# dgrzech/ir-sgmcmc

Measured on AMD Instinct MI355X. Metric: SG-MCMC transitions/sec (full _SGLD_transition), higher is better.
Workload: dtype f32; 1 GPU; 256^3 synthetic pair, SVF_3D 12 steps, GMM(K=4)/LCC(s=1) + virtual decimation, RegLoss_L2 w=1.4, Sobolev s=3, uniform noise 0.1, SGLD lr 0.4, Philox noise; init=identity, chains=1, parallelism=1 independent chain(s)

## Files before the change

include/irsgmcmc.h:

```cpp
#ifndef IRSGMCMC_H
#define IRSGMCMC_H

#include <stddef.h>
#include <stdint.h>

#ifdef __cplusplus
extern "C" {
#endif
#pragma GCC visibility push(default)

#define IRS_MAX_COMPONENTS 8
#define IRS_MAX_CHAINS 8
#define IRS_MAX_HALF_WIDTH 4
#define IRS_MAX_LABELS 64
#define IRS_HAUSDORFF_MAX_PERCENTILES 4

enum { IRS_DATA_GMM_LCC = 0, IRS_DATA_SSD = 1 };
enum { IRS_REG_L2 = 0, IRS_REG_LOGNORMAL = 1, IRS_REG_STUDENT = 2, IRS_REG_LOGNORMAL_L2 = 3 };


int irs_perturb_smooth(const float* v, const float* sigma, const float* eps, float tau, const float* kernel, int s,
                       int C, int D, int H, int W, float* tmp, float* out, uint64_t seed, uint64_t iteration,
                       void* stream);

// ... 242 lines not shown
void irs_destroy(irs_ctx* ctx);
size_t irs_workspace_bytes(const irs_ctx* ctx);
int irs_velocity_dims(const irs_ctx* ctx, int32_t out[3]);

int irs_set_fixed(irs_ctx* ctx, const float* fixed_im, int fixed_chains, void* stream);
int irs_get_state(irs_ctx* ctx, irs_state* out, void* stream);
int irs_set_state(irs_ctx* ctx, const irs_state* in, void* stream);
int irs_get_scalars(irs_ctx* ctx, irs_scalars* out, void* stream);

int irs_gmm_init(irs_ctx* ctx, const irs_io* io, const float* v_sample, int warm_up, void* stream);

int irs_transition(irs_ctx* ctx, const irs_io* io, void* stream);

int irs_flush(irs_ctx* ctx, void* stream);
int irs_recovered_transitions(const irs_ctx* ctx, uint64_t* out);

typedef struct irs_timings {
    float total_ms;
    float exp_fwd_ms;
    float exp_bwd_kernel_ms;
    float exp_bwd_total_ms;
    float smooth_ms;
    float data_ms;
    float update_ms;
    float exp_bwd_primary_avg_ms;
} irs_timings;
int irs_transition_timed(irs_ctx* ctx, const irs_io* io, void* stream, irs_timings* out);

typedef struct irs_comm irs_comm;
#define IRS_COMM_ID_BYTES 128
// ... 95 lines not shown
```

ir_sgmcmc_amd/_lib.py:

```python
import ctypes as C
import os

import torch

_HERE = os.path.dirname(os.path.abspath(__file__))
LIB_PATH = os.environ.get('IRS_LIB') or os.path.join(_HERE, 'csrc', 'libirsgmcmc.so')

IRS_MAX_COMPONENTS = 8
IRS_MAX_CHAINS = 8
IRS_MAX_HALF_WIDTH = 4
IRS_MAX_LABELS = 64
IRS_HAUSDORFF_MAX_PERCENTILES = 4
IRS_LABEL_BINS = 10
IRS_JACOBIAN_SUMMARY_INTS, IRS_JACOBIAN_SUMMARY_FLOATS = 4, 5
IRS_JACOBIAN_WS_BYTES = 1024 * (IRS_JACOBIAN_SUMMARY_INTS + IRS_JACOBIAN_SUMMARY_FLOATS) * 8
IRS_COVARIANCE_SUMMARY_INTS, IRS_COVARIANCE_SUMMARY_FLOATS = 2, 8
IRS_COVARIANCE_WS_BYTES = 1024 * (IRS_COVARIANCE_SUMMARY_INTS + IRS_COVARIANCE_SUMMARY_FLOATS) * 8
IRS_QUANTILE_MIN_BINS, IRS_QUANTILE_MAX_BINS, IRS_QUANTILE_MAX_PROBS, IRS_QUANTILE_MAX_RECORDS = 4, 256, 8, 65535
IRS_QUANTILE_SUMMARY_INTS, IRS_QUANTILE_SUMMARY_FLOATS = 3, 5
IRS_QUANTILE_WS_BYTES = 1024 * (IRS_QUANTILE_SUMMARY_INTS + IRS_QUANTILE_SUMMARY_FLOATS) * 8
IRS_ICE_SUMMARY_INTS, IRS_ICE_SUMMARY_FLOATS = 2, 3
IRS_ICE_WS_BYTES = IRS_MAX_CHAINS * 1024 * (IRS_ICE_SUMMARY_INTS + IRS_ICE_SUMMARY_FLOATS) * 8
IRS_ICE_MAP_SUMMARY_INTS, IRS_ICE_MAP_SUMMARY_FLOATS = 3, 3
IRS_ICE_MAP_WS_BYTES = 1024 * (IRS_ICE_MAP_SUMMARY_INTS + IRS_ICE_MAP_SUMMARY_FLOATS) * 8
# ... 159 lines not shown
                             C.c_size_t, _P],
    'irs_local_similarity_update': [_P, _I, _I, _I, _I, _P, _P, _P, _I, _P],
    'irs_local_similarity_finalize': [_P, _P, _P, _P, _I, _I, _I, _P, _P, _P, C.c_size_t, _P],
    'irs_create': [C.POINTER(IrsConfig), C.POINTER(_P)],
    'irs_destroy': [_P],
    'irs_workspace_bytes': [_P],
    'irs_velocity_dims': [_P, C.POINTER(C.c_int32 * 3)],
    'irs_set_fixed': [_P, _P, _I, _P],
    'irs_get_state': [_P, C.POINTER(IrsState), _P],
    'irs_set_state': [_P, C.POINTER(IrsState), _P],
    'irs_get_scalars': [_P, C.POINTER(IrsScalars), _P],
    'irs_gmm_init': [_P, C.POINTER(IrsIO), _P, _I, _P],
    'irs_transition': [_P, C.POINTER(IrsIO), _P],
    'irs_flush': [_P, _P],
    'irs_recovered_transitions': [_P, C.POINTER(C.c_uint64)],
    'irs_transition_timed': [_P, C.POINTER(IrsIO), _P, C.POINTER(IrsTimings)],
    'irs_comm_unique_id': [C.POINTER(C.c_uint8 * IRS_COMM_ID_BYTES)],
    'irs_comm_create_rccl': [C.POINTER(C.c_uint8 * IRS_COMM_ID_BYTES), _I, _I, C.POINTER(_P)],
    'irs_comm_create_ipc': [C.c_char_p, _I, _I, C.POINTER(_P)],
    'irs_comm_create_callbacks': [EXCHANGE_FN, ALLREDUCE_FN, _P, _I, _I, C.POINTER(_P)],
    'irs_comm_destroy': [_P],
    'irs_comm_probe': [_P, C.c_size_t, C.c_size_t, _I, _P, C.POINTER(C.c_double * 2)],
    'irs_comm_describe': [_P, C.c_char_p, C.c_size_t],
    'irs_comm_rank': [_P],
    'irs_comm_world': [_P],
    'irs_comm_selftest': [_P, _P],
    'irs_slab_plan_layout': [C.POINTER(IrsConfig), C.POINTER(IrsSlabConfig), _I, _I, C.POINTER(IrsSlabLayout)],
    'irs_slab_create': [C.POINTER(IrsConfig), C.POINTER(IrsSlabConfig), _P, C.POINTER(_P)],
    'irs_slab_get_layout': [_P, C.POINTER(IrsSlabLayout)],
    'irs_slab_transition': [_P, C.POINTER(IrsIO), _P],
# ... 65 lines not shown
```

ir_sgmcmc_amd/csrc/api_ctx.hip:

```cpp
#include <math.h>
#include <string.h>

#include <new>

#include "api_checks.h"
#include "comm.h"

using namespace irs;

static size_t align_up(size_t x) { return (x + 255) & ~(size_t)255; }

static bool is_capturing(hipStream_t st) {
    hipStreamCaptureStatus cap = hipStreamCaptureStatusNone;
    (void)hipStreamIsCapturing(st, &cap);
    return cap != hipStreamCaptureStatusNone;
}


int irs::create_ctx(const irs_config* cfg, const SlabInfo* sl, irs_ctx** out) {
    if (!cfg || !out) return fail("irs_create: null argument");
    const int D = cfg->dims[0], H = cfg->dims[1], W = cfg->dims[2], C = cfg->no_chains;
    if (!dims_ok(C, D, H, W) || !chain_count_ok(C)) return fail("irs_create: bad dims / chains (C <= %d)", IRS_MAX_CHAINS);
    if (cfg->no_steps < 1 || cfg->no_steps > 30) return fail("irs_create: no_steps out of range");
    if (cfg->sobolev_s < 0 || cfg->sobolev_s > IRS_MAX_HALF_WIDTH) return fail("irs_create: sobolev_s out of range");
// ... 4 lines not shown
    } else if (!(cfg->ssd_sigma > 0.0f)) return fail("irs_create: ssd_sigma must be positive");
    if (cfg->reg_loss < IRS_REG_L2 || cfg->reg_loss > IRS_REG_LOGNORMAL_L2) return fail("irs_create: unknown regulariser");
    if ((cfg->reg_loss == IRS_REG_STUDENT || cfg->reg_loss == IRS_REG_LOGNORMAL_L2) && cfg->reg_learnable)
        return fail("irs_create: RegLoss_Student / RegLoss_LogNormal_L2 have no learnable parameters");
    if (cfg->reg_loss == IRS_REG_STUDENT && !(cfg->w_reg_prior_rate > 0.0 && cfg->w_reg_prior_shape > 0.0))
        return fail("irs_create: RegLoss_Student needs a0 > 0 and b0 > 0 (w_reg_prior_shape / w_reg_prior_rate)");
    const bool any_cps = cfg->cps[0] || cfg->cps[1] || cfg->cps[2];
    if (any_cps && (cfg->cps[0] < 1 || cfg->cps[1] < 1 || cfg->cps[2] < 1 || cfg->cps[0] > 8 || cfg->cps[1] > 8 || cfg->cps[2] > 8))
        return fail("irs_create: control point spacing must be 1..8 on every axis");

    irs_ctx* c = new (std::nothrow) irs_ctx();
    if (!c) return fail("irs_create: out of host memory");
    memset((void*)c, 0, sizeof(*c));
    context_born();
    c->kn = global_knobs();
    c->cfg = *cfg;
    c->C = C;
    c->vol = make_vol(D, H, W);
    if (sl && sl->on) {
        c->sl = *sl;
        c->vol.V = (int64_t)(sl->hi - sl->lo) * H * W;
    }
    c->ffd = any_cps;
    c->volv = c->ffd ? make_vol(control_points(D, cfg->cps[0]), control_points(H, cfg->cps[1]), control_points(W, cfg->cps[2]))
                     : c->vol;
    c->sob.s = cfg->sobolev_s;
    for (int i = 0; i <= 2 * cfg->sobolev_s; ++i) c->sob.k[i] = cfg->sobolev_kernel[i];
    if (c->ffd)
        for (int a = 0; a < 3; ++a) c->spl[a] = make_spline(cfg->cps[a]);

// ... 39 lines not shown
    const size_t o_steps = take(fieldI * cfg->no_steps);
    const size_t o_tmpA = take(fieldV > ffd_tmp ? fieldV : ffd_tmp);
    const size_t o_tmpB = take(fieldV);
    const size_t o_vs = take(fieldV);
    const size_t o_gA = take(fieldI), o_gB = take(fieldI);
    const bool third = sl && sl->on && sl->world > 1;
    const size_t o_gC = third ? take(fieldI) : 0;
    const size_t o_warped = take(imageI), o_z = take(imageI), o_sig = take(imageI), o_fhat = take(imageI), o_gM = take(imageI);
    const size_t o_dense = take(c->ffd ? fieldI : 0);
    const size_t o_stat = take(sizeof(double) * kMaxPartialBlocks * kStatVals);
    const size_t o_energy = take(sizeof(double) * kMaxPartialBlocks * IRS_MAX_CHAINS);
    const size_t o_nll = take(sizeof(double) * (size_t)c->nll_blocks * C);
    const size_t o_sums = take(sizeof(double) * (kStatVals + 2 * IRS_MAX_CHAINS));
    const size_t o_dmax = take(sizeof(unsigned) * 4 * IRS_MAX_CHAINS * 32);
    const size_t o_cmm = take(coarse_minmax_bytes(c->vol, C));
    const size_t o_state = take(sizeof(DevState));
    c->slab_bytes = off;
    if (hipMalloc((void**)&c->slab, off) != hipSuccess) {
        irs_destroy(c);
        return fail("irs_create: hipMalloc of %zu workspace bytes failed", off);
    }
    if (c->sl.on) (void)hipMemset(c->slab, 0, off);
    c->steps = (float*)(c->slab + o_steps);
    c->tmpA = (float*)(c->slab + o_tmpA);
    c->tmpB = (float*)(c->slab + o_tmpB);
    c->vs = (float*)(c->slab + o_vs);
    c->gA = (float*)(c->slab + o_gA);
    c->gB = (float*)(c->slab + o_gB);
    c->gC = third ? (float*)(c->slab + o_gC) : nullptr;
    c->warped = (float*)(c->slab + o_warped);
    c->z = (float*)(c->slab + o_z);
    c->sigM = (float*)(c->slab + o_sig);
    c->fhat = (float*)(c->slab + o_fhat);
    c->gM = (float*)(c->slab + o_gM);
    c->dense = c->ffd ? (float*)(c->slab + o_dense) : nullptr;
    c->stat_partials = (double*)(c->slab + o_stat);
    c->energy_partials = (double*)(c->slab + o_energy);
    c->nll_partials = (double*)(c->slab + o_nll);
    c->stat_sum = (double*)(c->slab + o_sums);
    c->energy_sum = c->stat_sum + kStatVals;
    c->nll_sum = c->energy_sum + IRS_MAX_CHAINS;
    c->dmax = (unsigned*)(c->slab + o_dmax);
    c->cmm = (float*)(c->slab + o_cmm);
    c->state = (DevState*)(c->slab + o_state);

    if (ensure_lin_tables(c->lin, D, H, W, nullptr)) {
        irs_destroy(c);
        return fail("irs_create: identity grid allocation failed");
    }
    DevState init;
    memset(&init, 0, sizeof(init));
    init.K = d.K;
    init.mode = d.mode;
    init.ssd_inv_sigma = cfg->data_loss == IRS_DATA_SSD ? 1.0f / cfg->ssd_sigma : 0.0f;
    if (cfg->reg_loss == IRS_REG_L2 || cfg->reg_loss == IRS_REG_LOGNORMAL_L2) init.st.reg_param[0] = log((double)cfg->w_reg);
    for (int ch = 0; ch < IRS_MAX_CHAINS; ++ch) init.sc.alpha[ch] = 1.0;
    hipError_t e = hipMemcpy(c->state, &init, sizeof(init), hipMemcpyHostToDevice);
    if (e == hipSuccess) {
// ... 251 lines not shown
        if (overlap && ch + 1 < C) {
            HIP_TRY(hipEventRecord(c->ev_side[2 * ch], st));
            HIP_TRY(hipStreamWaitEvent(c->side, c->ev_side[2 * ch], 0));
            ds = c->side;
        }
        launch_data_bwd(cfg.data_loss, f, 0, zc, c->sigM + (int64_t)ch * vol.V, mask, 0, nullptr, c->state, ch,
                        c->gM + (int64_t)ch * vol.V, c->nll_partials + (int64_t)ch * c->nll_blocks, cfg.lcc_s, 1, vol, ds, c->nll_seg_C);
        if (ds != st) HIP_TRY(hipEventRecord(c->ev_side[2 * ch + 1], c->side));
    }
    if (batch)
        launch_data_bwd(cfg.data_loss, c->fhat, c->fhat_chains == 1 ? 0 : vol.V, z, c->sigM, io->mask, io->mask_chains == 1 ? 0 : vol.V, nullptr,
                        c->state, 0, c->gM, c->nll_partials, cfg.lcc_s, C, vol, st, c->nll_seg_C);
    if (!fuse_warp_bwd)
        launch_warp_bwd(io->moving_im, io->moving_chains == 1 ? 0 : vol.V, d_last, io->unif,
                        cfg.uniform_alpha > 0.0f ? cfg.uniform_alpha : 0.0f, c->gM, c->gA, C, vol, lin, cfg.seed, 0, it, st);
    LAUNCH_CHECK();
    if (timed) HIP_TRY(hipEventRecord(c->ev[3], st));
    const float* dense = c->ffd ? c->dense : vs;
    float* g0 = nullptr;
    {
        const float* G = c->gA;
        float* bufs[2] = {c->gB, c->gA};
        int cur = 0;
        for (int k = cfg.no_steps - 1; k >= 0; --k) {
            float* out = bufs[cur];
            const float* dk = k == 0 ? dense : c->steps + (int64_t)(k - 1) * field;
            if (timed) HIP_TRY(hipEventRecord(c->ev_bwd[2 * k], st));
            const unsigned* dm = c->dmax + (int64_t)k * C * 4;
            const float* gscale = fuse_warp_bwd && k == cfg.no_steps - 1 ? c->gM : nullptr;
            const int lay = bwd_lay(c, k) | (gscale ? 2 : 0);
            const bool sa = k < 32 && skip_any[k], s2 = k < 32 && skip_r2[k];
            const int gr = global_knobs().lds_from <= 2 ? 1 : 2;
            launch_exp_step_bwd_march(G, dk, out, k == 0, cfg.no_steps, C, vol, lin, dm, (s2 || (gr == 1 && !sa)) ? 1 : 2, sa, gscale, lay,
                                      timed ? c->ev_bwd[2 * k + 1] : nullptr, st);
            if (!sa) launch_exp_step_bwd_lds(G, dk, out, k == 0, cfg.no_steps, C, vol, lin, dm, 2, gr, gscale, lay, c->cmm, st);
            G = out;
            cur ^= 1;
        }
        g0 = const_cast<float*>(G);
    }
    if (timed) HIP_TRY(hipEventRecord(c->ev[4], st));
    float s[3];
    prescale_factors(vol, cfg.no_steps, s);
    if (c->ffd) {
        float* scaled = g0 == c->gA ? c->gB : c->gA;
        launch_scale_channels(g0, scaled, s[0], s[1], s[2], C, vol, st);
        const int G[3] = {volv.D, volv.H, volv.W};
        ffd_adjoint(scaled, c->tmpB, c->tmpA, C, vol, G, c->spl, st);
        launch_sgld_update(io->v, io->sigma, c->tmpB, vs, c->state, cfg.lr, 1.0f, 1.0f, 1.0f, io->grad_v, C, volv, st,
// ... 64 lines not shown
            if (enqueue_transition(c, &c->last_io, st, 0, true)) return 1;
        }
    }
    return fail("irs_flush: transitions keep failing");
}

int irs_flush(irs_ctx* c, void* stream) {
    if (!c) return fail("irs_flush: null argument");
    if (c->sl.on) return irs::slab_flush(c, (hipStream_t)stream);
    return flush_impl(c, (hipStream_t)stream);
}

int irs_recovered_transitions(const irs_ctx* c, uint64_t* out) {
    if (!c || !out) return fail("irs_recovered_transitions: null argument");
    *out = c->fails_total;
    return 0;
}

int irs_transition(irs_ctx* c, const irs_io* io, void* stream) { return transition_impl(c, io, (hipStream_t)stream, 0); }

int irs_transition_timed(irs_ctx* c, const irs_io* io, void* stream, irs_timings* out) {
    if (!out) return fail("irs_transition_timed: null output");
    if (c && c->cfg.no_steps > 32) return fail("irs_transition_timed: at most 32 steps");
    if (transition_impl(c, io, (hipStream_t)stream, 1)) return 1;
    HIP_TRY(hipEventSynchronize(c->ev[5]));
    memset(out, 0, sizeof(*out));
    HIP_TRY(hipEventElapsedTime(&out->total_ms, c->ev[0], c->ev[5]));
    HIP_TRY(hipEventElapsedTime(&out->smooth_ms, c->ev[0], c->ev[1]));
    HIP_TRY(hipEventElapsedTime(&out->exp_fwd_ms, c->ev[1], c->ev[2]));
    HIP_TRY(hipEventElapsedTime(&out->data_ms, c->ev[2], c->ev[3]));
// ... 13 lines not shown
```

ir_sgmcmc_amd/csrc/ctx.h:

```cpp
#pragma once
#include <stdlib.h>
#include <string.h>

#include "kernels.h"
#include "scalar_kernels.h"

struct irs_comm;

namespace irs {

int fail(const char* fmt, ...);

#define HIP_TRY(expr)                                                                               \
    do {                                                                                            \
        hipError_t e_ = (expr);                                                                     \
        if (e_ != hipSuccess) return irs::fail("%s failed: %s", #expr, hipGetErrorString(e_));      \
    } while (0)

#define LAUNCH_CHECK()                                                                              \
    do {                                                                                            \
        hipError_t e_ = hipGetLastError();                                                          \
        if (e_ != hipSuccess) return irs::fail("kernel launch failed: %s", hipGetErrorString(e_)); \
    } while (0)

// ... 14 lines not shown
struct irs_ctx {
    irs_config cfg;
    irs::DevCfg dcfg;
    irs::Vol vol, volv;
    bool ffd;
    int C;
    irs::LinTables lin;
    irs::Taps sob;
    irs::SplineTaps spl[3];
    char* slab;
    size_t slab_bytes;
    float *steps, *tmpA, *tmpB, *vs, *gA, *gB, *gC, *warped, *z, *sigM, *fhat, *gM, *dense;
    double *stat_partials, *energy_partials, *nll_partials;
    double *stat_sum, *energy_sum, *nll_sum;
    unsigned* dmax;
    float* cmm;
    unsigned* hint = nullptr;
    irs::DevState* state;
    int fhat_chains;
    bool fixed_set;
    int nll_blocks;
    int nll_seg_C;
    hipEvent_t ev[8];
    hipEvent_t ev_bwd[64];
    hipEvent_t ra_ev[4];
    hipStream_t side = nullptr;
    hipEvent_t ev_side[2 * IRS_MAX_CHAINS] = {};
    uint64_t n_enqueued = 0;
    irs::Knobs kn;
    bool dmax_clean = false;
// ... 119 lines not shown
```

ir_sgmcmc_amd/csrc/exp_kernels.hip:

```cpp
#include "kernels.h"

#include <type_traits>

namespace irs {

#ifndef IRS_ETX
#define IRS_ETX 32
#define IRS_ETY 8
#define IRS_ETZ 8
#endif
constexpr int ETX = IRS_ETX, ETY = IRS_ETY, ETZ = IRS_ETZ, ETN = ETX * ETY * ETZ;
constexpr int kExpBlock = 512;

struct Scale3L {
    float nm1[3];
    float rnm1[3];
    float inv_pow;
};

typedef float F3 __attribute__((ext_vector_type(3)));
__device__ __forceinline__ F3 ld3g(const float* __restrict__ p) {
    F3 v;
    __builtin_memcpy(&v, p, 12);
    return v;
// ... 725 lines not shown
    }
}

#ifdef IRS_BWD_TRACE
__device__ unsigned long long g_bwd_trace[8 * 64];
extern "C" __attribute__((visibility("default"))) int irs_debug_bwd_trace(unsigned long long* out) {
    return hipMemcpyFromSymbol(out, HIP_SYMBOL(g_bwd_trace), sizeof(g_bwd_trace)) == hipSuccess ? 0 : 1;
}
#define IRS_BT(slot)                                                                                  \
    do {                                                                                              \
        if (btrace_on && btrace_it < 64) g_bwd_trace[btrace_it * 8 + (slot)] = wall_clock64();        \
    } while (0)
#else
#define IRS_BT(slot)
#endif
template <bool PRESCALE, int R>
__device__ __forceinline__ void exp_bwd_march_tile(const float* __restrict__ G, const float* __restrict__ dk,
                                                   float* __restrict__ gout, const Vol vol, const Lin lin, const Scale3L sc,
                                                   const unsigned* __restrict__ dmax, const int seg_len, const int nseg,
                                                   const int r_lo, const int own_rest, const int swz_run, const int tile_id,
                                                   const dim3 tiles, const float* __restrict__ gscale, const int lay) {
    using M = March<PRESCALE, R>;
    constexpr int NP = M::NP, PX = M::PX, PN = M::PN, NIT = M::NIT;
    constexpr int NPQ = R == 2 ? 1 : NP;
    __shared__ float2 q_xy[NPQ * PN], q_zg[NPQ * PN], q_g[NPQ * PN], q_d[NP * PN];
    __shared__ float q_dz[NP * PN];
    const int tile_ = xcd_swizzle_runs(tile_id, (int)(tiles.x * tiles.y * tiles.z), swz_run);
    const int tbx = tile_ % tiles.x, tby = (tile_ / tiles.x) % tiles.y, tbz = tile_ / (tiles.x * tiles.y);
    const int chain = tbz / nseg, seg = tbz % nseg;
    const int hs = max(max((int)floorf(__uint_as_float(dmax[chain * 4 + 0])), (int)floorf(__uint_as_float(dmax[chain * 4 + 1]))),
                       (int)floorf(__uint_as_float(dmax[chain * 4 + 2]))) + 1;
    if (hs <= r_lo || (hs > R && !(R == 2 && own_rest))) return;
    const int ox = tbx * MTX, oy = tby * MTY;
    int z0, z1;
    seg_range(vol, seg, seg_len, z0, z1);
    const int64_t V = vol.V;
    const int64_t cb = (int64_t)chain * 3 * V;
    auto run = [&]() {
    const Lay3 LD = lay3(lay & 1, V), LG = lay3(lay & 2, V), LO = lay3(lay & 4, V);
    if (R == 2 && hs > R) {
        const int gx = ox + (int)(threadIdx.x % MTX), gy = oy + (int)(threadIdx.x / MTX);
        if (gx < vol.W && gy < vol.H)
            exp_bwd_generic_column<PRESCALE>(G + cb, LG, gscale ? gscale + (int64_t)chain * V : nullptr, dk + cb, LD, gout + cb, LO, vol,
                                             lin, sc, gx, gy, z0, z1, hs);
        return;
    }
    const float* __restrict__ dx_ = dk + cb;
    const float* __restrict__ dy_ = dx_ + LD.cs;
    const float* __restrict__ dz_ = dy_ + LD.cs;
    const float* __restrict__ Gx_ = G + cb;
// ... 263 lines not shown
    };
    run();
}

template <bool PRESCALE, int R>
__global__ __launch_bounds__(kMarchBlock, R == 1 ? IRS_MARCH_WAVES : IRS_MARCH_WAVES_R2) void exp_bwd_march_kernel(
    const float* __restrict__ G, const float* __restrict__ dk, float* __restrict__ gout, Vol vol, Lin lin, Scale3L sc,
    const unsigned* __restrict__ dmax, int seg_len, int nseg, int r_lo, int own_rest, int swz_run, dim3 tiles,
    const float* __restrict__ gscale, int lay) {
    const int total = (int)(tiles.x * tiles.y * tiles.z);
    for (int id = blockIdx.x; id < total; id += gridDim.x)
        exp_bwd_march_tile<PRESCALE, R>(G, dk, gout, vol, lin, sc, dmax, seg_len, nseg, r_lo, own_rest, swz_run, id, tiles, gscale, lay);
}


#ifndef IRS_BWD_MAX_SEG
#define IRS_BWD_MAX_SEG 64
#endif
constexpr int kRareGrid = 256 * IRS_MARCH_WAVES_R2;


void launch_exp_step_bwd_march(const float* G, const float* dk, float* gout, bool prescale_in, int no_steps, int C, Vol vol,
                               Lin lin, const unsigned* dmax, int max_radius, bool r2_owns_rest, const float* gscale, int lay,
                               hipEvent_t after_primary, hipStream_t st) {
    const int seg_env = global_knobs().march_seg;
    const int64_t per_layer = (int64_t)((vol.W + MTX - 1) / MTX) * ((vol.H + MTY - 1) / MTY) * C;
    int seg_len = pick_seg_len(vol.nz + vol.nzb, per_layer, 8, seg_env);
    if (global_knobs().seg_fit && seg_env <= 0) {
        static int cache = 0;
        const int64_t res = resident_blocks((const void*)exp_bwd_march_kernel<false, 1>, kMarchBlock, &cache);
        if (res > 0) seg_len = pick_seg_len_fit(vol.nz, vol.nzb, per_layer, 8, 2, res, 0, IRS_BWD_MAX_SEG);
    }
    const int nseg = vol_nseg(vol, seg_len);
    const dim3 tiles((vol.W + MTX - 1) / MTX, (vol.H + MTY - 1) / MTY, (unsigned)(nseg * C));
    const int total = (int)(tiles.x * tiles.y * tiles.z);
    const Scale3L sc = make_scale_l(vol, no_steps);
    const int swz_env = global_knobs().swz_run;
    const int swz_run = swz_env >= 0 ? swz_env : (int)tiles.x;
    if (global_knobs().launch_log) {
        static int cache_l = 0;
        log_launch("exp_bwd_march_kernel<R=1>", MTX, MTY, total, kMarchBlock, seg_len, 2, vol.nz + vol.nzb, C,
                   resident_blocks((const void*)exp_bwd_march_kernel<false, 1>, kMarchBlock, &cache_l));
    }
    auto launch = [&](auto P, auto RR, int r_lo, int grid, int seg, int nseg_, dim3 tiles_, int total_) {
        hipLaunchKernelGGL((exp_bwd_march_kernel<decltype(P)::value, decltype(RR)::value>), dim3(grid), dim3(kMarchBlock), 0, st, G, dk, gout, vol,
                           lin, sc, dmax, seg, nseg_, r_lo, r2_owns_rest ? 1 : 0, grid == total_ ? swz_run : 0, tiles_, gscale, lay);
    };
    with_bool(prescale_in, [&](auto P) { launch(P, Int<1>{}, 0, total, seg_len, nseg, tiles, total); });
    if (after_primary) (void)hipEventRecord(after_primary, st);
    if (max_radius >= 2) {
        int seg2 = seg_len;
        if (global_knobs().seg_fit && seg_env <= 0)
            seg2 = pick_seg_len_fit(vol.nz, vol.nzb, per_layer, 8, 4, kRareGrid, 0, IRS_BWD_MAX_SEG);
        const int nseg2 = vol_nseg(vol, seg2);
        const dim3 tiles2(tiles.x, tiles.y, (unsigned)(nseg2 * C));
        const int total2 = (int)(tiles2.x * tiles2.y * tiles2.z);
        const int rare = total2 < kRareGrid ? total2 : kRareGrid;
        with_bool(prescale_in, [&](auto P) { launch(P, Int<2>{}, 1, rare, seg2, nseg2, tiles2, total2); });
    }
}

#ifndef IRS_FTX
#define IRS_FTX 64
// ... 384 lines not shown
```

ir_sgmcmc_amd/csrc/kernels.h:

```cpp
#pragma once
#include "common.h"

namespace irs {

struct Taps {
    float k[2 * IRS_MAX_HALF_WIDTH + 1];
    int s;
};

struct SplineTaps {
    float k[32];
    int cps;
};

struct LinTables {
    float* dev = nullptr;
    int D = 0, H = 0, W = 0;
    Lin lin() const { return Lin{dev, dev + W, dev + W + H}; }
};
int ensure_lin_tables(LinTables& t, int D, int H, int W, hipStream_t st);
int cached_lin(int D, int H, int W, hipStream_t st, Lin* out);

void launch_perturb(const float* v, const float* sigma, const float* eps, float amp, float* out, int C, Vol vol,
                    uint64_t seed, uint64_t iteration, const uint64_t* dev_iteration, hipStream_t st);
// ... 5 lines not shown
void launch_warp_bwd(const float* im, int64_t im_stride, const float* d, const float* unif, float alpha,
                     const float* g_warped, float* g_d, int C, Vol vol, Lin lin, uint64_t seed, uint64_t iteration,
                     const uint64_t* dev_iteration, hipStream_t st);
void launch_warp_transformation(const float* im, int64_t im_stride, const float* t, float* out, int C, Vol vol,
                                hipStream_t st);
void launch_warp_nearest_u8(const uint8_t* im, int64_t im_stride, const float* t, uint8_t* out, int C, Vol vol,
                            hipStream_t st);
void launch_warp_nearest_i16(const int16_t* im, int64_t im_stride, const float* t, int16_t* out, int C, Vol vol,
                             hipStream_t st);
void launch_ffd_axis(const float* in, float* out, const SplineTaps& taps, bool adjoint, int64_t outer, int n_in,
                     int n_out, int64_t inner, hipStream_t st, int w_lo = 0, int w_n = -1, int store_lo = 0, int store_n = -1);
void launch_scale_channels(const float* in, float* out, float s0, float s1, float s2, int C, Vol vol, hipStream_t st);

void launch_exp_step_fwd_march(const float* din, float* dout, bool prescale, int no_steps, int C, Vol vol, Lin lin,
                               const unsigned* dmax_in, unsigned* dmax_out, bool only_r1, int lay, hipStream_t st);
void launch_exp_step_bwd_march(const float* G, const float* dk, float* gout, bool prescale, int no_steps, int C, Vol vol,
                               Lin lin, const unsigned* dmax, int max_radius, bool r2_owns_rest, const float* gscale, int lay,
                               hipEvent_t after_primary, hipStream_t st);
size_t coarse_minmax_bytes(Vol vol, int C);
void launch_exp_step_bwd_lds(const float* G, const float* dk, float* gout, bool prescale, int no_steps, int C, Vol vol,
                             Lin lin, const unsigned* dmax, int halo, int gather_radius, const float* gscale, int lay,
                             float* cmm, hipStream_t st);
void launch_field_absmax(const float* d, bool prescale, int no_steps, unsigned* dmax, int C, Vol vol, hipStream_t st);

void launch_sobolev_march(const float* in, float* out, const Taps& taps, int planes, Vol vol, unsigned* dmax0, int no_steps,
                          hipStream_t st);
void launch_perturb_sobolev_march(const float* v, const float* sigma, const float* eps, float amp, float* out, const Taps& taps,
                                  int C, Vol vol, unsigned* dmax0, int no_steps, uint64_t seed, uint64_t iteration,
                                  const uint64_t* dev_iteration, hipStream_t st);
void launch_lcc_fwd_march(const float* fhat, int64_t fhat_stride, const float* im, float* z, float* sigma_out, int s, int C,
                    Vol vol, hipStream_t st);
struct GmmDev;
void launch_data_bwd(int mode, const float* fhat_or_fixed, int64_t f_stride, const float* z, const float* sigma_m,
                     const uint8_t* mask, int64_t mask_stride, const float* g_z_override, const void* dev_state,
                     int chain, float* g_warped, double* nll_partials, int s, int C_launch, Vol vol, hipStream_t st, int seg_C = 1);
void launch_stats(int want_vd, const float* z, const uint8_t* mask, const void* dev_state, double* partials, Vol vol,
                  hipStream_t st, int K = 0);
void launch_residual_ssd(const float* fixed, int64_t f_stride, const float* warped, float* z, int C, Vol vol,
// ... 172 lines not shown
```

ir_sgmcmc_amd/engine.py:

```python
import ctypes as C
import math
from dataclasses import dataclass, field
from typing import Optional, Sequence, Tuple

import torch
from scipy.special import digamma

from . import _lib as L
from .ops import control_grid_size, sobolev_kernel_1d


@dataclass
class EngineConfig:
    dims: Tuple[int, int, int]
    no_chains: int = 1
    cps: Optional[Tuple[int, int, int]] = None
    no_steps: int = 12
    sobolev_s: int = 3
    sobolev_lambda: float = 0.5
    lr: float = 0.4
    uniform_noise: float = 0.1
    virtual_decimation: bool = True
    data_loss: str = 'GMM'
    gmm_components: int = 4
# ... 109 lines not shown
                pass

    def option(self, name, value):
        L.option_set(name, value, self._ctx)

    @_on_device
    def flush(self):
        L.check(self.lib.irs_flush(self._ctx, self._stream()))

    @property
    def recovered_transitions(self):
        n = C.c_uint64()
        L.check(self.lib.irs_recovered_transitions(self._ctx, C.byref(n)))
        return int(n.value)

    @property
    def workspace_bytes(self):
        return int(self.lib.irs_workspace_bytes(self._ctx))

    @_on_device
    def state(self):
        st = L.IrsState()
        L.check(self.lib.irs_get_state(self._ctx, C.byref(st), self._stream()))
        return st

    @_on_device
    def set_state(self, st):
        L.check(self.lib.irs_set_state(self._ctx, C.byref(st), self._stream()))

    @_on_device
# ... 52 lines not shown
```

Before: 231.3 transitions/s.

## Add sparse adjoint plan to skip zero-gradient columns in SVF backward march

Adds a planning pass that finds, per xy tile column and scaling-squaring step, the z range where the warped-image gradient is nonzero, widened by the displacement bound. The backward march kernel then processes only planned pieces from a work list and zero-fills the remaining regions, falling back to dense handling when displacements are large. It aims to cut adjoint work where the gradient is spatially sparse, for example where a mask limits it, at the cost of extra planning kernels, a memset and more workspace.

```diff
diff --git a/include/irsgmcmc.h b/include/irsgmcmc.h
--- a/include/irsgmcmc.h
+++ b/include/irsgmcmc.h
@@ -280,6 +280,8 @@
 
 int irs_flush(irs_ctx* ctx, void* stream);
 int irs_recovered_transitions(const irs_ctx* ctx, uint64_t* out);
+int irs_sparse_adjoint_set(irs_ctx* ctx, int on);
+int irs_sparse_adjoint_get(irs_ctx* ctx, int32_t* out, void* stream);
 
 typedef struct irs_timings {
     float total_ms;
diff --git a/ir_sgmcmc_amd/_lib.py b/ir_sgmcmc_amd/_lib.py
--- a/ir_sgmcmc_amd/_lib.py
+++ b/ir_sgmcmc_amd/_lib.py
@@ -197,6 +197,8 @@
     'irs_transition': [_P, C.POINTER(IrsIO), _P],
     'irs_flush': [_P, _P],
     'irs_recovered_transitions': [_P, C.POINTER(C.c_uint64)],
+    'irs_sparse_adjoint_set': [_P, _I],
+    'irs_sparse_adjoint_get': [_P, _I32P, _P],
     'irs_transition_timed': [_P, C.POINTER(IrsIO), _P, C.POINTER(IrsTimings)],
     'irs_comm_unique_id': [C.POINTER(C.c_uint8 * IRS_COMM_ID_BYTES)],
     'irs_comm_create_rccl': [C.POINTER(C.c_uint8 * IRS_COMM_ID_BYTES), _I, _I, C.POINTER(_P)],
diff --git a/ir_sgmcmc_amd/csrc/adjoint_plan.h b/ir_sgmcmc_amd/csrc/adjoint_plan.h
--- /dev/null
+++ b/ir_sgmcmc_amd/csrc/adjoint_plan.h
@@ -0,0 +1,102 @@
+#pragma once
+
+#if defined(__HIPCC__)
+#define IRS_HD __host__ __device__ inline
+#else
+#define IRS_HD inline
+#endif
+
+namespace irs {
+
+#ifndef IRS_MTX
+#define IRS_MTX 32
+#define IRS_MTY 8
+#endif
+constexpr int kPlanTX = IRS_MTX, kPlanTY = IRS_MTY;
+#ifndef IRS_BWD_MAX_SEG
+#define IRS_BWD_MAX_SEG 64
+#endif
+constexpr int kPlanMaxLen = IRS_BWD_MAX_SEG;
+constexpr int kPlanMinLen = 8;
+constexpr int kPlanMinForced = 4;
+constexpr int kPlanStats = 4;
+
+struct PlanEntry {
+    int chain, tile, z0, z1, fill, pad;
+};
+
+struct ColPlan {
+    int lo, hi, f0, f1;
+};
+
+IRS_HD int plan_min(int a, int b) { return a < b ? a : b; }
+IRS_HD int plan_max(int a, int b) { return a > b ? a : b; }
+
+IRS_HD void plan_widen(int a, int b, int m, int D, int& lo, int& hi) {
+    lo = hi = 0;
+    if (b <= 0) return;
+    lo = plan_max(D - a - m, 0);
+    hi = plan_min(b + m, D);
+}
+
+IRS_HD ColPlan plan_column(int lo, int hi, int nlo, int nhi) {
+    const bool run = hi > lo, need = nhi > nlo;
+    if (!run) return need ? ColPlan{nhi, nhi, nlo, nhi} : ColPlan{0, 0, 0, 0};
+    return ColPlan{lo, hi, need ? plan_min(lo, nlo) : lo, need ? plan_max(hi, nhi) : hi};
+}
+
+IRS_HD ColPlan plan_column_of(const int* runs, int k, int col, int C, int ntx, int nty, int D) {
+    const int tiles = ntx * nty, chain = col / tiles, tile = col - chain * tiles, tx = tile % ntx, ty = tile / ntx;
+    const int* r = runs + ((long long)k * C * tiles + col) * 2;
+    int nlo = 0, nhi = D;
+    if (k > 0) {
+        nlo = D;
+        nhi = 0;
+        const int* prev = runs + ((long long)(k - 1) * C + chain) * tiles * 2;
+        for (int dy = -1; dy <= 1; ++dy)
+            for (int dx = -1; dx <= 1; ++dx) {
+                const int ux = plan_min(plan_max(tx + dx, 0), ntx - 1), uy = plan_min(plan_max(ty + dy, 0), nty - 1);
+                const int l = prev[(uy * ntx + ux) * 2], h = prev[(uy * ntx + ux) * 2 + 1];
+                if (h > l) {
+                    nlo = plan_min(nlo, plan_max(l - 1, 0));
+                    nhi = plan_max(nhi, plan_min(h + 1, D));
+                }
+            }
+    }
+    return plan_column(r[0], r[1], nlo, nhi);
+}
+
+IRS_HD int plan_pieces(int len, int L) { return len > 0 ? (len + L - 1) / L : 0; }
+
+IRS_HD void plan_cut(int lo, int len, int np, int j, int& z0, int& z1) {
+    z0 = lo + (int)((long long)len * j / np);
+    z1 = lo + (int)((long long)len * (j + 1) / np);
+}
+
+IRS_HD PlanEntry plan_entry(const ColPlan& c, int chain, int tile, int np, int j) {
+    int z0, z1;
+    plan_cut(c.lo, c.hi - c.lo, np, j, z0, z1);
+    return PlanEntry{chain, tile, z0, z1, 0, 0};
+}
+IRS_HD bool plan_has_fill(const ColPlan& c, int side) { return side == 0 ? c.f0 < c.lo : c.hi < c.f1 && c.hi > c.lo; }
+IRS_HD PlanEntry plan_fill_entry(const ColPlan& c, int chain, int tile, int side) {
+    return side == 0 ? PlanEntry{chain, tile, c.f0, c.lo, 1, 0} : PlanEntry{chain, tile, c.hi, c.f1, 1, 0};
+}
+
+IRS_HD int plan_pick_len(const int* pieces, int G, int lmin, int lmax) {
+    for (int L = lmin; L < lmax; ++L)
+        if (pieces[L] <= G) return L;
+    return lmax;
+}
+
+IRS_HD int plan_entries_cap(int columns, int D) { return columns * ((D + kPlanMinForced - 1) / kPlanMinForced + 2); }
+
+IRS_HD int plan_swizzle(int id, int count, int run) {
+    if (run <= 1) return id;
+    const int group = 8 * run;
+    if (id >= count / group * group) return id;
+    const int g = id / group, w = id - g * group;
+    return g * group + (w & 7) * run + (w >> 3);
+}
+
+}
diff --git a/ir_sgmcmc_amd/csrc/adjoint_plan.hip b/ir_sgmcmc_amd/csrc/adjoint_plan.hip
--- /dev/null
+++ b/ir_sgmcmc_amd/csrc/adjoint_plan.hip
@@ -0,0 +1,218 @@
+#include "adjoint_plan.h"
+
+#include "kernels.h"
+
+namespace irs {
+
+constexpr int kExtChunk = 32;
+
+__global__ __launch_bounds__(kBlock) void grad_extent_kernel(const float* __restrict__ g, int* __restrict__ ext, Vol vol) {
+    const int x = (int)blockIdx.x * 64 + ((int)threadIdx.x & 63), y = (int)blockIdx.y * 4 + ((int)threadIdx.x >> 6);
+    const int nch = (vol.D + kExtChunk - 1) / kExtChunk;
+    const int chain = (int)blockIdx.z / nch, za = ((int)blockIdx.z - chain * nch) * kExtChunk, zb = min(za + kExtChunk, vol.D);
+    if (x >= vol.W || y >= vol.H) return;
+    const int64_t plane = (int64_t)vol.H * vol.W;
+    const float* __restrict__ p = g + (int64_t)chain * vol.V + (int64_t)y * vol.W + x;
+    int lo = vol.D, hi = -1;
+#pragma unroll 8
+    for (int z = za; z < zb; ++z) {
+        const bool nz = p[z * plane] != 0.0f;
+        lo = nz ? min(lo, z) : lo;
+        hi = nz ? z : hi;
+    }
+    if (hi < 0) return;
+    int* e = ext + ((int64_t)chain * plane + (int64_t)y * vol.W + x) * 2;
+    atomicMax(e, vol.D - lo);
+    atomicMax(e + 1, hi + 1);
+}
+
+__device__ __forceinline__ bool chain_is_dense(const unsigned* __restrict__ dmax, int chain, int C, int no_steps) {
+    bool dense = false;
+    for (int k = 0; k < no_steps; ++k) {
+        const unsigned* b = dmax + ((int64_t)k * C + chain) * 4;
+        const float m = fmaxf(fmaxf(__uint_as_float(b[0]), __uint_as_float(b[1])), __uint_as_float(b[2]));
+        dense |= !(m < 1.0f);
+    }
+    return dense;
+}
+
+__global__ __launch_bounds__(kWave) void plan_runs_kernel(const int* __restrict__ ext, const unsigned* __restrict__ dmax,
+                                                          int* __restrict__ runs, Vol vol, int C, int no_steps, int ntx, int nty) {
+    const int col = (int)blockIdx.x, k = (int)blockIdx.y, tiles = ntx * nty;
+    const int chain = col / tiles, tile = col - chain * tiles, tx = tile % ntx, ty = tile / ntx;
+    int* out = runs + ((int64_t)k * C * tiles + col) * 2;
+    if (chain_is_dense(dmax, chain, C, no_steps)) {
+        if (threadIdx.x == 0) {
+            out[0] = 0;
+            out[1] = vol.D;
+        }
+        return;
+    }
+    const int m = no_steps - k;
+    const int x0 = max(tx * kPlanTX - m, 0), x1 = min(tx * kPlanTX + kPlanTX + m, vol.W);
+    const int y0 = max(ty * kPlanTY - m, 0), y1 = min(ty * kPlanTY + kPlanTY + m, vol.H);
+    const int nx = x1 - x0, n = nx * (y1 - y0);
+    const int* __restrict__ e = ext + (int64_t)chain * vol.H * vol.W * 2;
+    int lo = vol.D, hi = 0;
+    for (int i = (int)threadIdx.x; i < n; i += kWave) {
+        const int yy = i / nx, xx = i - yy * nx;
+        const int2 ab = *reinterpret_cast<const int2*>(e + ((int64_t)(y0 + yy) * vol.W + x0 + xx) * 2);
+        int l, h;
+        plan_widen(ab.x, ab.y, m, vol.D, l, h);
+        if (h > l) {
+            lo = min(lo, l);
+            hi = max(hi, h);
+        }
+    }
+#pragma unroll
+    for (int off = kWave / 2; off > 0; off >>= 1) {
+        lo = min(lo, __shfl_xor(lo, off, kWave));
+        hi = max(hi, __shfl_xor(hi, off, kWave));
+    }
+    if (threadIdx.x == 0) {
+        out[0] = hi > lo ? lo : 0;
+        out[1] = hi > lo ? hi : 0;
+    }
+}
+
+constexpr int kPlanBlock = 1024;
+__device__ __forceinline__ int block_rank(bool flag, int* wave_tot, int& total) {
+    const unsigned long long b = __ballot(flag);
+    const int lane = (int)threadIdx.x & (kWave - 1), w = (int)threadIdx.x / kWave;
+    if (lane == 0) wave_tot[w] = __popcll(b);
+    __syncthreads();
+    int before = 0;
+    total = 0;
+#pragma unroll
+    for (int i = 0; i < kPlanBlock / kWave; ++i) {
+        before += i < w ? wave_tot[i] : 0;
+        total += wave_tot[i];
+    }
+    __syncthreads();
+    return before + __popcll(b & ((1ull << lane) - 1ull));
+}
+
+__global__ __launch_bounds__(kPlanBlock) void plan_lists_kernel(const int* __restrict__ runs, const unsigned* __restrict__ dmax,
+                                                                ColPlan* __restrict__ colplan, PlanEntry* __restrict__ entries,
+                                                                int* __restrict__ count, int* __restrict__ stats, Vol vol, int C,
+                                                                int no_steps, int ntx, int nty, int cap, int G, int forced_len) {
+    __shared__ int pieces[kPlanMaxLen + 1], s_maxlen, s_L, wave_tot[kPlanBlock / kWave];
+    __shared__ int s_pieces[IRS_MAX_CHAINS], s_planes[IRS_MAX_CHAINS];
+    const int k = (int)blockIdx.x, tiles = ntx * nty, cols = C * tiles, tid = (int)threadIdx.x;
+    const int lmax = max(min(kPlanMaxLen, vol.D), 1), lmin = min(kPlanMinLen, lmax);
+    ColPlan* __restrict__ cps = colplan + (int64_t)k * cols;
+    for (int i = tid; i <= kPlanMaxLen; i += kPlanBlock) pieces[i] = 0;
+    if (tid < IRS_MAX_CHAINS) s_pieces[tid] = s_planes[tid] = 0;
+    if (tid == 0) s_maxlen = 0;
+    __syncthreads();
+    for (int col = tid; col < cols; col += kPlanBlock) {
+        const ColPlan cp = plan_column_of(runs, k, col, C, ntx, nty, vol.D);
+        cps[col] = cp;
+        const int len = cp.hi - cp.lo;
+        if (len > 0) {
+            atomicMax(&s_maxlen, len);
+            atomicAdd(&s_planes[col / tiles], len);
+        }
+    }
+    __syncthreads();
+    const int n_len = lmax - lmin + 1, groups = kPlanBlock / n_len;
+    if (forced_len <= 0 && tid < groups * n_len) {
+        const int L = lmin + tid % n_len;
+        int sum = 0;
+        for (int col = tid / n_len; col < cols; col += groups) sum += plan_pieces(cps[col].hi - cps[col].lo, L);
+        atomicAdd(&pieces[L], sum);
+    }
+    __syncthreads();
+    if (tid == 0) s_L = forced_len > 0 ? min(max(forced_len, kPlanMinForced), lmax) : plan_pick_len(pieces, G, lmin, lmax);
+    __syncthreads();
+    const int L = s_L, levels = plan_pieces(s_maxlen, L);
+    PlanEntry* list = entries + (int64_t)k * cap;
+    int base = 0, n_run = 0;
+    for (int j = 0; j < levels + 2; ++j)
+        for (int c0 = 0; c0 < cols; c0 += kPlanBlock) {
+            const int col = c0 + tid;
+            bool flag = false;
+            ColPlan cp = {0, 0, 0, 0};
+            int np = 0;
+            if (col < cols) {
+                cp = cps[col];
+                np = plan_pieces(cp.hi - cp.lo, L);
+                flag = j < levels ? j < np : plan_has_fill(cp, j - levels);
+            }
+            int total;
+            const int pos = base + block_rank(flag, wave_tot, total);
+            if (flag && pos < cap) {
+                list[pos] = j < levels ? plan_entry(cp, col / tiles, col % tiles, np, j) : plan_fill_entry(cp, col / tiles, col % tiles, j - levels);
+                atomicAdd(&s_pieces[col / tiles], 1);
+            }
+            base += total;
+            if (j < levels) n_run = base;
+        }
+    __syncthreads();
+    if (tid == 0) {
+        count[2 * k] = min(base, cap);
+        count[2 * k + 1] = min(n_run, cap);
+    }
+    if (tid < C) {
+        int* s = stats + ((int64_t)k * C + tid) * kPlanStats;
+        s[0] = chain_is_dense(dmax, tid, C, no_steps) ? 0 : 1;
+        s[1] = L;
+        s[2] = s_pieces[tid];
+        s[3] = s_planes[tid];
+    }
+}
+
+static size_t plan_align(size_t b) { return (b + 255) / 256 * 256; }
+
+struct PlanLayout {
+    size_t ext, runs, colplan, entries, count, stats, total;
+    int cap, ntx, nty;
+};
+static PlanLayout plan_layout(Vol vol, int C, int no_steps) {
+    PlanLayout l;
+    l.ntx = (vol.W + kPlanTX - 1) / kPlanTX;
+    l.nty = (vol.H + kPlanTY - 1) / kPlanTY;
+    const size_t cols = (size_t)C * l.ntx * l.nty;
+    l.cap = plan_entries_cap((int)cols, vol.D);
+    size_t off = 0;
+    auto take = [&](size_t bytes) { const size_t o = off; off += plan_align(bytes); return o; };
+    l.ext = take(sizeof(int) * 2 * (size_t)C * vol.H * vol.W);
+    l.runs = take(sizeof(int) * 2 * cols * no_steps);
+    l.colplan = take(sizeof(ColPlan) * cols * no_steps);
+    l.entries = take(sizeof(PlanEntry) * (size_t)l.cap * no_steps);
+    l.count = take(sizeof(int) * 2 * no_steps);
+    l.stats = take(sizeof(int) * kPlanStats * (size_t)C * no_steps);
+    l.total = off;
+    return l;
+}
+
+size_t adjoint_plan_bytes(Vol vol, int C, int no_steps) { return plan_layout(vol, C, no_steps).total; }
+
+AdjointPlan adjoint_plan_views(char* base, Vol vol, int C, int no_steps) {
+    const PlanLayout l = plan_layout(vol, C, no_steps);
+    AdjointPlan p;
+    p.ext = (int*)(base + l.ext);
+    p.runs = (int*)(base + l.runs);
+    p.colplan = (ColPlan*)(base + l.colplan);
+    p.entries = (PlanEntry*)(base + l.entries);
+    p.count = (int*)(base + l.count);
+    p.stats = (int*)(base + l.stats);
+    p.cap = l.cap;
+    p.ntx = l.ntx;
+    p.nty = l.nty;
+    return p;
+}
+
+void launch_adjoint_plan(const float* g_warped, const unsigned* dmax, const AdjointPlan& plan, int no_steps, int C, Vol vol,
+                         int64_t G, int forced_len, hipStream_t st) {
+    (void)hipMemsetAsync(plan.ext, 0, sizeof(int) * 2 * (size_t)C * vol.H * vol.W, st);
+    const int nch = (vol.D + kExtChunk - 1) / kExtChunk;
+    hipLaunchKernelGGL(grad_extent_kernel, dim3((unsigned)((vol.W + 63) / 64), (unsigned)((vol.H + 3) / 4), (unsigned)(nch * C)), dim3(kBlock),
+                       0, st, g_warped, plan.ext, vol);
+    hipLaunchKernelGGL(plan_runs_kernel, dim3((unsigned)(C * plan.ntx * plan.nty), (unsigned)no_steps), dim3(kWave), 0, st, plan.ext, dmax,
+                       plan.runs, vol, C, no_steps, plan.ntx, plan.nty);
+    hipLaunchKernelGGL(plan_lists_kernel, dim3((unsigned)no_steps), dim3(kPlanBlock), 0, st, plan.runs, dmax, plan.colplan, plan.entries, plan.count,
+                       plan.stats, vol, C, no_steps, plan.ntx, plan.nty, plan.cap, (int)(G > 0 ? G : 1024), forced_len);
+}
+
+}
diff --git a/ir_sgmcmc_amd/csrc/api_ctx.hip b/ir_sgmcmc_amd/csrc/api_ctx.hip
--- a/ir_sgmcmc_amd/csrc/api_ctx.hip
+++ b/ir_sgmcmc_amd/csrc/api_ctx.hip
@@ -3,6 +3,7 @@
 
 #include <new>
 
+#include "adjoint_plan.h"
 #include "api_checks.h"
 #include "comm.h"
 
@@ -42,6 +43,7 @@
     memset((void*)c, 0, sizeof(*c));
     context_born();
     c->kn = global_knobs();
+    c->sparse_adjoint = true;
     c->cfg = *cfg;
     c->C = C;
     c->vol = make_vol(D, H, W);
@@ -111,6 +113,8 @@
     const size_t o_sums = take(sizeof(double) * (kStatVals + 2 * IRS_MAX_CHAINS));
     const size_t o_dmax = take(sizeof(unsigned) * 4 * IRS_MAX_CHAINS * 32);
     const size_t o_cmm = take(coarse_minmax_bytes(c->vol, C));
+    const bool planned = !sl;
+    const size_t o_plan = take(planned ? adjoint_plan_bytes(c->vol, C, cfg->no_steps) : 0);
     const size_t o_state = take(sizeof(DevState));
     c->slab_bytes = off;
     if (hipMalloc((void**)&c->slab, off) != hipSuccess) {
@@ -139,6 +143,7 @@
     c->nll_sum = c->energy_sum + IRS_MAX_CHAINS;
     c->dmax = (unsigned*)(c->slab + o_dmax);
     c->cmm = (float*)(c->slab + o_cmm);
+    if (planned) c->plan = adjoint_plan_views(c->slab + o_plan, c->vol, C, cfg->no_steps);
     c->state = (DevState*)(c->slab + o_state);
 
     if (ensure_lin_tables(c->lin, D, H, W, nullptr)) {
@@ -420,6 +425,10 @@
     if (!fuse_warp_bwd)
         launch_warp_bwd(io->moving_im, io->moving_chains == 1 ? 0 : vol.V, d_last, io->unif,
                         cfg.uniform_alpha > 0.0f ? cfg.uniform_alpha : 0.0f, c->gM, c->gA, C, vol, lin, cfg.seed, 0, it, st);
+    const bool sparse = c->sparse_adjoint && c->plan.entries != nullptr &&
+                        (global_knobs().march_seg > 0 || exp_bwd_dense_seg_len(vol, C) > kPlanMinLen);
+    c->plan_on = sparse;
+    if (sparse) launch_adjoint_plan(c->gM, c->dmax, c->plan, cfg.no_steps, C, vol, exp_bwd_plan_resident(), global_knobs().march_seg, st);
     LAUNCH_CHECK();
     if (timed) HIP_TRY(hipEventRecord(c->ev[3], st));
     const float* dense = c->ffd ? c->dense : vs;
@@ -438,7 +447,7 @@
             const bool sa = k < 32 && skip_any[k], s2 = k < 32 && skip_r2[k];
             const int gr = global_knobs().lds_from <= 2 ? 1 : 2;
             launch_exp_step_bwd_march(G, dk, out, k == 0, cfg.no_steps, C, vol, lin, dm, (s2 || (gr == 1 && !sa)) ? 1 : 2, sa, gscale, lay,
-                                      timed ? c->ev_bwd[2 * k + 1] : nullptr, st);
+                                      timed ? c->ev_bwd[2 * k + 1] : nullptr, st, sparse ? &c->plan : nullptr, k);
             if (!sa) launch_exp_step_bwd_lds(G, dk, out, k == 0, cfg.no_steps, C, vol, lin, dm, 2, gr, gscale, lay, c->cmm, st);
             G = out;
             cur ^= 1;
@@ -533,6 +542,23 @@
 int irs_recovered_transitions(const irs_ctx* c, uint64_t* out) {
     if (!c || !out) return fail("irs_recovered_transitions: null argument");
     *out = c->fails_total;
+    return 0;
+}
+
+int irs_sparse_adjoint_set(irs_ctx* c, int on) {
+    if (!c) return fail("irs_sparse_adjoint_set: null argument");
+    c->sparse_adjoint = on != 0;
+    return 0;
+}
+
+int irs_sparse_adjoint_get(irs_ctx* c, int32_t* out, void* stream) {
+    if (!c || !out) return fail("irs_sparse_adjoint_get: null argument");
+    const size_t n = (size_t)c->cfg.no_steps * c->C * kPlanStats;
+    memset(out, 0, n * sizeof(int32_t));
+    if (!c->plan.stats || !c->plan_on || c->n_enqueued == 0) return 0;
+    if (irs_flush(c, stream)) return 1;
+    HIP_TRY(hipMemcpyAsync(out, c->plan.stats, n * sizeof(int32_t), hipMemcpyDeviceToHost, (hipStream_t)stream));
+    HIP_TRY(hipStreamSynchronize((hipStream_t)stream));
     return 0;
 }
 
diff --git a/ir_sgmcmc_amd/csrc/ctx.h b/ir_sgmcmc_amd/csrc/ctx.h
--- a/ir_sgmcmc_amd/csrc/ctx.h
+++ b/ir_sgmcmc_amd/csrc/ctx.h
@@ -52,6 +52,9 @@
     double *stat_partials, *energy_partials, *nll_partials;
     double *stat_sum, *energy_sum, *nll_sum;
     unsigned* dmax;
+    irs::AdjointPlan plan;
+    bool sparse_adjoint = true;
+    bool plan_on = false;
     float* cmm;
     unsigned* hint = nullptr;
     irs::DevState* state;
diff --git a/ir_sgmcmc_amd/csrc/exp_kernels.hip b/ir_sgmcmc_amd/csrc/exp_kernels.hip
--- a/ir_sgmcmc_amd/csrc/exp_kernels.hip
+++ b/ir_sgmcmc_amd/csrc/exp_kernels.hip
@@ -1,3 +1,4 @@
+#include "adjoint_plan.h"
 #include "kernels.h"
 
 #include <type_traits>
@@ -763,26 +764,32 @@
 #else
 #define IRS_BT(slot)
 #endif
-template <bool PRESCALE, int R>
+template <bool PRESCALE, int R, bool PLAN = false>
 __device__ __forceinline__ void exp_bwd_march_tile(const float* __restrict__ G, const float* __restrict__ dk,
                                                    float* __restrict__ gout, const Vol vol, const Lin lin, const Scale3L sc,
                                                    const unsigned* __restrict__ dmax, const int seg_len, const int nseg,
                                                    const int r_lo, const int own_rest, const int swz_run, const int tile_id,
-                                                   const dim3 tiles, const float* __restrict__ gscale, const int lay) {
+                                                   const dim3 tiles, const float* __restrict__ gscale, const int lay,
+                                                   const PlanEntry piece = PlanEntry{}) {
     using M = March<PRESCALE, R>;
     constexpr int NP = M::NP, PX = M::PX, PN = M::PN, NIT = M::NIT;
     constexpr int NPQ = R == 2 ? 1 : NP;
     __shared__ float2 q_xy[NPQ * PN], q_zg[NPQ * PN], q_g[NPQ * PN], q_d[NP * PN];
     __shared__ float q_dz[NP * PN];
-    const int tile_ = xcd_swizzle_runs(tile_id, (int)(tiles.x * tiles.y * tiles.z), swz_run);
+    const int tile_ = PLAN ? piece.tile : xcd_swizzle_runs(tile_id, (int)(tiles.x * tiles.y * tiles.z), swz_run);
     const int tbx = tile_ % tiles.x, tby = (tile_ / tiles.x) % tiles.y, tbz = tile_ / (tiles.x * tiles.y);
-    const int chain = tbz / nseg, seg = tbz % nseg;
+    const int chain = PLAN ? piece.chain : tbz / nseg, seg = tbz % nseg;
     const int hs = max(max((int)floorf(__uint_as_float(dmax[chain * 4 + 0])), (int)floorf(__uint_as_float(dmax[chain * 4 + 1]))),
                        (int)floorf(__uint_as_float(dmax[chain * 4 + 2]))) + 1;
     if (hs <= r_lo || (hs > R && !(R == 2 && own_rest))) return;
     const int ox = tbx * MTX, oy = tby * MTY;
     int z0, z1;
-    seg_range(vol, seg, seg_len, z0, z1);
+    if (PLAN) {
+        z0 = piece.z0;
+        z1 = piece.z1;
+    } else {
+        seg_range(vol, seg, seg_len, z0, z1);
+    }
     const int64_t V = vol.V;
     const int64_t cb = (int64_t)chain * 3 * V;
     auto run = [&]() {
@@ -1076,15 +1083,53 @@
 }
 
 
-#ifndef IRS_BWD_MAX_SEG
-#define IRS_BWD_MAX_SEG 64
-#endif
+constexpr int kPlanFillBlocks = 256;
+__device__ __forceinline__ void plan_zero_fill(float* __restrict__ o, const Lay3 LO, const Vol vol, const int ox, const int oy, int za, int zb) {
+    za = max(za, 0);
+    zb = min(zb, vol.D);
+    const int lx = threadIdx.x % MTX, ly = threadIdx.x / MTX;
+    const int x = ox + lx, y = oy + ly;
+    if (!(x < vol.W && y < vol.H)) return;
+    const unsigned g = (unsigned)(y * vol.W + x) * 4u * (unsigned)LO.em;
+    for (int z = za; z < zb; ++z) {
+        const int64_t pl = (int64_t)z * vol.H * vol.W * LO.em;
+        if (LO.em == 3) {
+            st3_off(o + pl, g, 0.0f, 0.0f, 0.0f);
+        } else {
+            st_off(o + pl, g, 0.0f);
+            st_off(o + LO.cs + pl, g, 0.0f);
+            st_off(o + 2 * LO.cs + pl, g, 0.0f);
+        }
+    }
+}
+template <bool PRESCALE>
+__global__ __launch_bounds__(kMarchBlock, IRS_MARCH_WAVES) void exp_bwd_march_plan_kernel(
+    const float* __restrict__ G, const float* __restrict__ dk, float* __restrict__ gout, Vol vol, Lin lin, Scale3L sc,
+    const unsigned* __restrict__ dmax, const PlanEntry* __restrict__ entries, const int* __restrict__ count, int swz_run, dim3 tiles,
+    const float* __restrict__ gscale, int lay) {
+    const int n = count[0], n_run = count[1];
+    if (blockIdx.x < kPlanFillBlocks) {
+        for (int id = n_run + (int)blockIdx.x; id < n; id += kPlanFillBlocks) {
+            const PlanEntry e = entries[id];
+            plan_zero_fill(gout + (int64_t)e.chain * 3 * vol.V, lay3(lay & 4, vol.V), vol, (e.tile % (int)tiles.x) * MTX,
+                           (e.tile / (int)tiles.x) * MTY, e.z0, e.z1);
+        }
+        return;
+    }
+    const int first = (int)blockIdx.x - kPlanFillBlocks, stride = (int)gridDim.x - kPlanFillBlocks;
+    for (int id = first; id < n_run; id += stride)
+        exp_bwd_march_tile<PRESCALE, 1, true>(G, dk, gout, vol, lin, sc, dmax, 0, 1, 0, 0, 0, id, tiles, gscale, lay,
+                                              entries[plan_swizzle(id, n_run, swz_run)]);
+}
+int64_t exp_bwd_plan_resident() {
+    static int cache = 0;
+    return resident_blocks((const void*)exp_bwd_march_plan_kernel<false>, kMarchBlock, &cache);
+}
+
 constexpr int kRareGrid = 256 * IRS_MARCH_WAVES_R2;
 
 
-void launch_exp_step_bwd_march(const float* G, const float* dk, float* gout, bool prescale_in, int no_steps, int C, Vol vol,
-                               Lin lin, const unsigned* dmax, int max_radius, bool r2_owns_rest, const float* gscale, int lay,
-                               hipEvent_t after_primary, hipStream_t st) {
+int exp_bwd_dense_seg_len(Vol vol, int C) {
     const int seg_env = global_knobs().march_seg;
     const int64_t per_layer = (int64_t)((vol.W + MTX - 1) / MTX) * ((vol.H + MTY - 1) / MTY) * C;
     int seg_len = pick_seg_len(vol.nz + vol.nzb, per_layer, 8, seg_env);
@@ -1093,6 +1138,15 @@
         const int64_t res = resident_blocks((const void*)exp_bwd_march_kernel<false, 1>, kMarchBlock, &cache);
         if (res > 0) seg_len = pick_seg_len_fit(vol.nz, vol.nzb, per_layer, 8, 2, res, 0, IRS_BWD_MAX_SEG);
     }
+    return seg_len;
+}
+
+void launch_exp_step_bwd_march(const float* G, const float* dk, float* gout, bool prescale_in, int no_steps, int C, Vol vol,
+                               Lin lin, const unsigned* dmax, int max_radius, bool r2_owns_rest, const float* gscale, int lay,
+                               hipEvent_t after_primary, hipStream_t st, const AdjointPlan* plan, int step) {
+    const int seg_env = global_knobs().march_seg;
+    const int64_t per_layer = (int64_t)((vol.W + MTX - 1) / MTX) * ((vol.H + MTY - 1) / MTY) * C;
+    const int seg_len = exp_bwd_dense_seg_len(vol, C);
     const int nseg = vol_nseg(vol, seg_len);
     const dim3 tiles((vol.W + MTX - 1) / MTX, (vol.H + MTY - 1) / MTY, (unsigned)(nseg * C));
     const int total = (int)(tiles.x * tiles.y * tiles.z);
@@ -1108,7 +1162,17 @@
         hipLaunchKernelGGL((exp_bwd_march_kernel<decltype(P)::value, decltype(RR)::value>), dim3(grid), dim3(kMarchBlock), 0, st, G, dk, gout, vol,
                            lin, sc, dmax, seg, nseg_, r_lo, r2_owns_rest ? 1 : 0, grid == total_ ? swz_run : 0, tiles_, gscale, lay);
     };
-    with_bool(prescale_in, [&](auto P) { launch(P, Int<1>{}, 0, total, seg_len, nseg, tiles, total); });
+    if (plan && vol.nzb == 0 && vol.z0 == 0 && vol.nz == vol.D) {
+        const int64_t res = exp_bwd_plan_resident();
+        const dim3 tiles2d(tiles.x, tiles.y, 1);
+        with_bool(prescale_in, [&](auto P) {
+            hipLaunchKernelGGL((exp_bwd_march_plan_kernel<decltype(P)::value>), dim3((unsigned)((res > 0 ? res : kExpGridCap) + kPlanFillBlocks)), dim3(kMarchBlock), 0,
+                               st, G, dk, gout, vol, lin, sc, dmax, plan->entries + (int64_t)step * plan->cap, plan->count + 2 * step, swz_run, tiles2d,
+                               gscale, lay);
+        });
+    } else {
+        with_bool(prescale_in, [&](auto P) { launch(P, Int<1>{}, 0, total, seg_len, nseg, tiles, total); });
+    }
     if (after_primary) (void)hipEventRecord(after_primary, st);
     if (max_radius >= 2) {
         int seg2 = seg_len;
diff --git a/ir_sgmcmc_amd/csrc/kernels.h b/ir_sgmcmc_amd/csrc/kernels.h
--- a/ir_sgmcmc_amd/csrc/kernels.h
+++ b/ir_sgmcmc_amd/csrc/kernels.h
@@ -43,14 +43,33 @@
 
 void launch_exp_step_fwd_march(const float* din, float* dout, bool prescale, int no_steps, int C, Vol vol, Lin lin,
                                const unsigned* dmax_in, unsigned* dmax_out, bool only_r1, int lay, hipStream_t st);
+struct AdjointPlan;
 void launch_exp_step_bwd_march(const float* G, const float* dk, float* gout, bool prescale, int no_steps, int C, Vol vol,
                                Lin lin, const unsigned* dmax, int max_radius, bool r2_owns_rest, const float* gscale, int lay,
-                               hipEvent_t after_primary, hipStream_t st);
+                               hipEvent_t after_primary, hipStream_t st, const AdjointPlan* plan = nullptr, int step = 0);
+int exp_bwd_dense_seg_len(Vol vol, int C);
+int64_t exp_bwd_plan_resident();
 size_t coarse_minmax_bytes(Vol vol, int C);
 void launch_exp_step_bwd_lds(const float* G, const float* dk, float* gout, bool prescale, int no_steps, int C, Vol vol,
                              Lin lin, const unsigned* dmax, int halo, int gather_radius, const float* gscale, int lay,
                              float* cmm, hipStream_t st);
 void launch_field_absmax(const float* d, bool prescale, int no_steps, unsigned* dmax, int C, Vol vol, hipStream_t st);
+
+struct PlanEntry;
+struct ColPlan;
+struct AdjointPlan {
+    int* ext = nullptr;
+    int* runs = nullptr;
+    ColPlan* colplan = nullptr;
+    PlanEntry* entries = nullptr;
+    int* count = nullptr;
+    int* stats = nullptr;
+    int cap = 0, ntx = 0, nty = 0;
+};
+size_t adjoint_plan_bytes(Vol vol, int C, int no_steps);
+AdjointPlan adjoint_plan_views(char* base, Vol vol, int C, int no_steps);
+void launch_adjoint_plan(const float* g_warped, const unsigned* dmax, const AdjointPlan& plan, int no_steps, int C, Vol vol,
+                         int64_t G, int forced_len, hipStream_t st);
 
 void launch_sobolev_march(const float* in, float* out, const Taps& taps, int planes, Vol vol, unsigned* dmax0, int no_steps,
                           hipStream_t st);
diff --git a/ir_sgmcmc_amd/engine.py b/ir_sgmcmc_amd/engine.py
--- a/ir_sgmcmc_amd/engine.py
+++ b/ir_sgmcmc_amd/engine.py
@@ -147,6 +147,17 @@
         L.check(self.lib.irs_recovered_transitions(self._ctx, C.byref(n)))
         return int(n.value)
 
+    def set_sparse_adjoint(self, on):
+        L.check(self.lib.irs_sparse_adjoint_set(self._ctx, int(bool(on))))
+
+    @_on_device
+    def sparse_adjoint(self):
+        n, ch = self.cfg.no_steps, self.cfg.no_chains
+        buf = (C.c_int32 * (n * ch * 4))()
+        L.check(self.lib.irs_sparse_adjoint_get(self._ctx, buf, self._stream()))
+        keys = ('engaged', 'piece_len', 'pieces', 'run_planes')
+        return [[dict(zip(keys, buf[(k * ch + c) * 4:(k * ch + c) * 4 + 4])) for c in range(ch)] for k in range(n)]
+
     @property
     def workspace_bytes(self):
         return int(self.lib.irs_workspace_bytes(self._ctx))
```

Result: faster. 254.7 transitions/s (median of 6 runs) (+10.1%).
